# sine2pi/ASR-model

Measured on AMD Instinct MI355X. Metric: audio-sec/sec fwd+bwd on 30s@16kHz LibriSpeech-shaped clips (whole job, all GPUs), higher is better.
Workload: dtype bf16; 1 GPU; tiny (BASELINE configs[1]): log-mel + 4 enc/4 dec d=384 h=6 fwd+bwd, 32 x 30 s clips per GPU, T=256; model=tiny, global_batch=32, seq_len=3001, text_len=256, pitch_frames=3001, parallelism=dp1

## Files before the change

### asr-model_amd/csrc/gemm_wn.hip

```cpp
#include "gemm_wr.h"
#include "gemm_p2.h"
#include "gemm_ws.h"
#include <string>

static int g_wide_variant = 5;
static bool ws_on() { return (g_wide_variant & 4) != 0; }
static bool ws_any() { return (g_wide_variant & 8) != 0; }
extern "C" int asrx_set_gemm_variant(int v) {
  const int old = g_wide_variant;
  g_wide_variant = v;
  return old;
}
static bool p2_ok(const asrx::wn::Params& p, int conv, int nj, int a_bf16) {
  if (!a_bf16 && p.M >= 131072) return false;
  const bool vec = ((p.N | p.ldc) & 3) == 0 && ((uintptr_t)p.C & 15) == 0 && ((uintptr_t)p.Z & 15) == 0 &&
                   ((uintptr_t)p.Cb & 7) == 0;
  return (g_wide_variant & 3) >= 1 && !conv && (nj == 3 || nj == 2 || (nj == 1 && (g_wide_variant & 3) == 2)) &&
         vec && p.K >= 64;
}

namespace asrx {
namespace wn {

__global__ void weight_to_bf16_kernel(const float* __restrict__ src, unsigned short* __restrict__ dst, int rows,
                                      int cols, int64_t ld, int trans) {
  const int64_t total = (int64_t)rows * cols;
  for (int64_t i = (int64_t)blockIdx.x * blockDim.x + threadIdx.x; i < total; i += (int64_t)gridDim.x * blockDim.x) {
    int64_t r, c, o;
    if (!trans) {
      r = i / cols;
      c = i % cols;
      o = r * cols + c;
    } else {
      c = i / rows;
      r = i % rows;
      o = c * rows + r;
    }
    __bf16 h = (__bf16)src[r * ld + c];
    dst[o] = __builtin_bit_cast(unsigned short, h);
  }
}

}
}

using namespace asrx;

extern "C" int asrx_weight_to_bf16(const float* src, unsigned short* dst, int64_t rows, int64_t cols, int64_t ld,
                                   int trans, hipStream_t stream) {
  if (rows * cols == 0) return 0;
  const int64_t n = rows * cols;
  wn::weight_to_bf16_kernel<<<(unsigned)std::min<int64_t>((n + 255) / 256, 16384), 256, 0, stream>>>(
      src, dst, (int)rows, (int)cols, ld, trans);
  ASRX_LAUNCHED("asrx_weight_to_bf16");
}

struct WConv {
  const float* src;
  unsigned short* dst;
  int64_t ld;
  int rows, cols, trans, pad;
};

namespace asrx {
__global__ __launch_bounds__(256) void weights_to_bf16_kernel(const WConv* __restrict__ tab) {
  const WConv e = tab[blockIdx.y];
  const int64_t total = (int64_t)e.rows * e.cols;
  const int64_t i0 = (int64_t)blockIdx.x * 4096;
  if (i0 >= total) return;
  const int64_t i1 = min<int64_t>(total, i0 + 4096);
  for (int64_t i = i0 + threadIdx.x; i < i1; i += 256) {
    int64_t r, c, o;
    if (!e.trans) {
      r = i / e.cols;
      c = i % e.cols;
      o = r * e.cols + c;
    } else {
      c = i / e.rows;
      r = i % e.rows;
      o = c * e.rows + r;
    }
    e.dst[o] = __builtin_bit_cast(unsigned short, (__bf16)e.src[r * e.ld + c]);
  }
}
}

extern "C" int64_t asrx_wconv_entry_bytes(void) { return (int64_t)sizeof(WConv); }

extern "C" int asrx_weights_to_bf16(const void* tab, int64_t n, int64_t max_elems, hipStream_t stream) {
  if (n == 0) return 0;
  ASRX_REQUIRE(n < 65536, "asrx_weights_to_bf16: too many entries");
  dim3 grid((unsigned)((max_elems + 4095) / 4096), (unsigned)n);
  weights_to_bf16_kernel<<<grid, 256, 0, stream>>>((const WConv*)tab);
  ASRX_LAUNCHED("asrx_weights_to_bf16");
}

extern "C" int asrx_gemm_wn(const float* A, int64_t lda, int conv, int64_t convF, int64_t convC,
                            const unsigned short* W, int64_t ldw, float* C, int64_t ldc, const float* bias, float* Z,
                            int64_t M, int64_t N, int64_t K, float alpha, float beta, int act, int nj,
                            hipStream_t stream) {
  ASRX_REQUIRE(M > 0 && N > 0 && K > 0, "asrx_gemm_wn: empty problem");
  ASRX_REQUIRE(((uintptr_t)A & 15) == 0 && ((uintptr_t)W & 15) == 0, "asrx_gemm_wn: A/W must be 16-byte aligned");
  ASRX_REQUIRE(K % 8 == 0 && lda % 4 == 0 && ldw % 8 == 0, "asrx_gemm_wn: K%%8, lda%%4, ldw%%8 required");
  ASRX_REQUIRE(M * lda < (1LL << 31) && N * ldw < (1LL << 31), "asrx_gemm_wn: operand spans >= 2^31 elements");
  ASRX_REQUIRE(!conv || (convF > 0 && convC % 4 == 0), "asrx_gemm_wn: conv needs F > 0 and C %% 4 == 0");
  wn::Params p{A, (int)lda, W, (int)ldw, C, (int)ldc, bias, Z, (int)M, (int)N, (int)K,
               (int)(convF > 0 ? convF : 1), (int)(convC > 0 ? convC : 1), alpha, beta, act, nullptr, nullptr};
  if (nj == 3) conv ? wn::launch_wr<3, true>(p, stream) : wn::launch_wr<3, false>(p, stream);
  else if (nj == 2) conv ? wn::launch_wr<2, true>(p, stream) : wn::launch_wr<2, false>(p, stream);
  else conv ? wn::launch_wr<1, true>(p, stream) : wn::launch_wr<1, false>(p, stream);
  ASRX_LAUNCHED("asrx_gemm_wn");
}

extern "C" int asrx_gemm_wn_ex(const void* A, int a_bf16, int64_t lda, int conv, int64_t convF, int64_t convC,
                               const unsigned short* W, int64_t ldw, void* C, int c_bf16, int64_t ldc,
                               const float* bias, float* Z, int64_t M, int64_t N, int64_t K, float alpha, float beta,
                               int act, int nj, const int* mtiles, const int* n_mtiles, hipStream_t stream) {
  ASRX_REQUIRE(M > 0 && N > 0 && K > 0, "asrx_gemm_wn_ex: empty problem");
  ASRX_REQUIRE(((uintptr_t)A & 15) == 0 && ((uintptr_t)W & 15) == 0, "asrx_gemm_wn_ex: A/W must be 16-byte aligned");
  ASRX_REQUIRE(K % 8 == 0 && lda % (a_bf16 ? 8 : 4) == 0 && ldw % 8 == 0,
               "asrx_gemm_wn_ex: K%%8, lda%%4 (fp32) / lda%%8 (bf16), ldw%%8 required");
  ASRX_REQUIRE(M * lda < (1LL << 31) && N * ldw < (1LL << 31), "asrx_gemm_wn_ex: operand spans >= 2^31 elements");
  ASRX_REQUIRE(!conv || (convF > 0 && convC % (a_bf16 ? 8 : 4) == 0), "asrx_gemm_wn_ex: conv needs F > 0 and C %% 4 (8 for bf16)");
  ASRX_REQUIRE(!c_bf16 || beta == 0.f, "asrx_gemm_wn_ex: a bf16 output takes beta = 0");
  ASRX_REQUIRE(!(conv && mtiles), "asrx_gemm_wn_ex: tile lists are for plain GEMMs");
  wn::Params p{(const float*)A, (int)lda, W, (int)ldw, c_bf16 ? nullptr : (float*)C, (int)ldc, bias, Z, (int)M,
               (int)N, (int)K, (int)(convF > 0 ? convF : 1), (int)(convC > 0 ? convC : 1), alpha, beta, act,
               nullptr, nullptr, mtiles, n_mtiles, c_bf16 ? (unsigned short*)C : nullptr};
#define ASRX_WN_EX(NJV)                                                                              \
  if (a_bf16) conv ? wn::launch_wr<NJV, true, false, true>(p, stream) : wn::launch_wr<NJV, false, false, true>(p, stream); \
  else conv ? wn::launch_wr<NJV, true>(p, stream) : wn::launch_wr<NJV, false>(p, stream);
  if (ws_on() && !conv && wn::ws_ok(p, a_bf16, ws_any())) {
    a_bf16 ? wn::launch_ws_act<true>(p, stream) : wn::launch_ws_act<false>(p, stream);
  } else if (p2_ok(p, conv, nj, a_bf16)) {
    if (nj == 3) a_bf16 ? wn::launch_p2_act<3, true, false>(p, stream) : wn::launch_p2_act<3, false, false>(p, stream);
    else a_bf16 ? wn::launch_p2_act<2, true, false>(p, stream) : wn::launch_p2_act<2, false, false>(p, stream);
  } else if (nj == 3) { ASRX_WN_EX(3) }
  else if (nj == 2) { ASRX_WN_EX(2) }
  else { ASRX_WN_EX(1) }
#undef ASRX_WN_EX
  ASRX_LAUNCHED("asrx_gemm_wn_ex");
}

extern "C" int asrx_gemm_wn_ce(const void* A, int64_t lda, const unsigned short* W, int64_t ldw, unsigned short* Zb,
                               int64_t ldc, float* part, int64_t M, int64_t N, int64_t K, int nj, hipStream_t stream) {
  ASRX_REQUIRE(M > 0 && N > 0 && K > 0, "asrx_gemm_wn_ce: empty problem");
  ASRX_REQUIRE(((uintptr_t)A & 15) == 0 && ((uintptr_t)W & 15) == 0 && ((uintptr_t)Zb & 7) == 0 &&
                   ((uintptr_t)part & 7) == 0,
               "asrx_gemm_wn_ce: A/W 16-byte, Zb/part 8-byte aligned");
  ASRX_REQUIRE(K % 8 == 0 && lda % 8 == 0 && ldw % 8 == 0 && N % 4 == 0 && ldc % 4 == 0,
               "asrx_gemm_wn_ce: K, lda, ldw %% 8 and N, ldc %% 4 required");
  ASRX_REQUIRE(M * lda < (1LL << 31) && N * ldw < (1LL << 31), "asrx_gemm_wn_ce: operand spans >= 2^31 elements");
  ASRX_REQUIRE(nj >= 1 && nj <= 3, "asrx_gemm_wn_ce: nj in 1..3");
  wn::Params p{(const float*)A, (int)lda, W, (int)ldw, nullptr, (int)ldc, nullptr, nullptr, (int)M, (int)N, (int)K,
               1, 1, 1.f, 0.f, ACT_NONE, nullptr, nullptr, nullptr, nullptr, Zb, (float2*)part,
               (int)((N + 128 * nj - 1) / (128 * nj))};
  if (nj == 3) wn::launch_wr<3, false, false, true, true>(p, stream);
  else if (nj == 2) wn::launch_wr<2, false, false, true, true>(p, stream);
  else wn::launch_wr<1, false, false, true, true>(p, stream);
  ASRX_LAUNCHED("asrx_gemm_wn_ce");
}

extern "C" int asrx_gemm_wn_ce_f32(const void* A, int64_t lda, const unsigned short* W, int64_t ldw, float* Zf,
                               int64_t ldc, float* part, int64_t M, int64_t N, int64_t K, int nj, hipStream_t stream) {
  ASRX_REQUIRE(M > 0 && N > 0 && K > 0, "asrx_gemm_wn_ce_f32: empty problem");
  ASRX_REQUIRE(((uintptr_t)A & 15) == 0 && ((uintptr_t)W & 15) == 0 && ((uintptr_t)Zf & 15) == 0 &&
                   ((uintptr_t)part & 7) == 0,
               "asrx_gemm_wn_ce_f32: A/W 16-byte, Zf 16-byte, part 8-byte aligned");
  ASRX_REQUIRE(K % 8 == 0 && lda % 8 == 0 && ldw % 8 == 0 && N % 4 == 0 && ldc % 4 == 0,
               "asrx_gemm_wn_ce_f32: K, lda, ldw %% 8 and N, ldc %% 4 required");
  ASRX_REQUIRE(M * lda < (1LL << 31) && N * ldw < (1LL << 31), "asrx_gemm_wn_ce_f32: operand spans >= 2^31 elements");
  ASRX_REQUIRE(nj >= 1 && nj <= 3, "asrx_gemm_wn_ce_f32: nj in 1..3");
  wn::Params p{(const float*)A, (int)lda, W, (int)ldw, Zf, (int)ldc, nullptr, nullptr, (int)M, (int)N, (int)K,
               1, 1, 1.f, 0.f, ACT_NONE, nullptr, nullptr, nullptr, nullptr, nullptr, (float2*)part,
               (int)((N + 128 * nj - 1) / (128 * nj))};
  if (nj == 3) wn::launch_wr<3, false, false, true, true>(p, stream);
  else if (nj == 2) wn::launch_wr<2, false, false, true, true>(p, stream);
  else wn::launch_wr<1, false, false, true, true>(p, stream);
  ASRX_LAUNCHED("asrx_gemm_wn_ce_f32");
}

extern "C" int asrx_gemm_wn_head(const void* A, int64_t lda, const unsigned short* W, int64_t ldw, float* part,
                                 const int64_t* labels, float* zlab, int64_t M, int64_t N, int64_t K, int nj,
                                 hipStream_t stream) {
  ASRX_REQUIRE(M > 0 && N > 0 && K > 0, "asrx_gemm_wn_head: empty problem");
  ASRX_REQUIRE(((uintptr_t)A & 15) == 0 && ((uintptr_t)W & 15) == 0 && ((uintptr_t)part & 7) == 0,
               "asrx_gemm_wn_head: A/W 16-byte, part 8-byte aligned");
  ASRX_REQUIRE(K % 8 == 0 && lda % 8 == 0 && ldw % 8 == 0 && N % 4 == 0 && lda >= K,
               "asrx_gemm_wn_head: K, lda, ldw %% 8, N %% 4 and lda >= K required");
  ASRX_REQUIRE(M * lda < (1LL << 31) && N * ldw < (1LL << 31), "asrx_gemm_wn_head: operand spans >= 2^31 elements");
  ASRX_REQUIRE(nj >= 1 && nj <= 3, "asrx_gemm_wn_head: nj in 1..3");
  ASRX_REQUIRE(!labels || zlab, "asrx_gemm_wn_head: labels need zlab");
  const int64_t nparts = (N + 128 * nj - 1) / (128 * nj);
  wn::Params p{(const float*)A, (int)lda, W, (int)ldw, nullptr, (int)N, nullptr, nullptr, (int)M, (int)N, (int)K,
               1, 1, 1.f, 0.f, ACT_NONE, nullptr, nullptr, nullptr, nullptr, nullptr, (float2*)part, (int)nparts};
  p.hd_idx = reinterpret_cast<int*>(part + 2 * M * nparts);
  p.hd_labels = labels;
  p.hd_zlab = zlab;
  if (nj == 3) wn::launch_wr<3, false, false, true, true, false, false, false, true>(p, stream);
  else if (nj == 2) wn::launch_wr<2, false, false, true, true, false, false, false, true>(p, stream);
  else wn::launch_wr<1, false, false, true, true, false, false, false, true>(p, stream);
  ASRX_LAUNCHED("asrx_gemm_wn_head");
}

extern "C" int asrx_gemm_wn_res(const float* A, int64_t lda, const unsigned short* W, int64_t ldw, float* C, int64_t ldc,
                                const float* bias, const float* R, int64_t ldr, int64_t M, int64_t N, int64_t K, int nj,
                                hipStream_t stream) {
  ASRX_REQUIRE(M > 0 && N > 0 && K > 0, "asrx_gemm_wn_res: empty problem");
  ASRX_REQUIRE(((uintptr_t)A & 15) == 0 && ((uintptr_t)W & 15) == 0 && ((uintptr_t)C & 15) == 0 &&
                   ((uintptr_t)R & 15) == 0,
               "asrx_gemm_wn_res: A/W/C/R must be 16-byte aligned");
  ASRX_REQUIRE(K % 8 == 0 && lda % 4 == 0 && ldw % 8 == 0 && N % 4 == 0 && ldc % 4 == 0 && ldr % 4 == 0,
               "asrx_gemm_wn_res: K, ldw %% 8; lda, N, ldc, ldr %% 4");
  ASRX_REQUIRE(M * lda < (1LL << 31) && N * ldw < (1LL << 31), "asrx_gemm_wn_res: operand spans >= 2^31 elements");
  ASRX_REQUIRE(R && R != C, "asrx_gemm_wn_res: a residual input distinct from C is required");
  ASRX_REQUIRE(nj == 1 || nj == 3, "asrx_gemm_wn_res: nj 1 or 3");
  wn::Params p{A, (int)lda, W, (int)ldw, C, (int)ldc, bias, nullptr, (int)M, (int)N, (int)K, 1, 1, 1.f, 0.f,
               ACT_NONE, nullptr, nullptr, nullptr, nullptr, nullptr, nullptr, 0, R, (int)ldr};
  if (ws_on() && wn::ws_ok(p, false, ws_any())) wn::launch_ws<false, ACT_NONE, true, false>(p, stream);
  else if (nj == 3 && p2_ok(p, 0, nj, 0)) wn::launch_p2_act<3, false, true>(p, stream);
  else if (nj == 3) wn::launch_wr<3, false, false, false, false, true>(p, stream);
  else wn::launch_wr<1, false, false, false, false, true>(p, stream);
  ASRX_LAUNCHED("asrx_gemm_wn_res");
}

extern "C" int asrx_gemm_wn_rot(const void* A, int a_bf16, int64_t lda, const unsigned short* W, int64_t ldw,
                                float* C, float* Z, int64_t ldc, const float* bias, const float* m, const float* tab,
                                int64_t L, int64_t hd, float scale, int64_t M, int64_t N, int64_t K, int nj,
                                hipStream_t stream) {
  ASRX_REQUIRE(M > 0 && N > 0 && K > 0 && L > 0, "asrx_gemm_wn_rot: empty problem");
  ASRX_REQUIRE(((uintptr_t)A & 15) == 0 && ((uintptr_t)W & 15) == 0 && ((uintptr_t)C & 15) == 0 &&
                   ((uintptr_t)Z & 15) == 0 && ((uintptr_t)tab & 15) == 0,
               "asrx_gemm_wn_rot: A/W/C/Z/tab must be 16-byte aligned");
  ASRX_REQUIRE(K % 8 == 0 && lda % (a_bf16 ? 8 : 4) == 0 && ldw % 8 == 0 && N % 4 == 0 && ldc % 4 == 0,
               "asrx_gemm_wn_rot: K, ldw %% 8; lda %% 4 (8 bf16); N, ldc %% 4");
  ASRX_REQUIRE(hd >= 4 && hd % 4 == 0 && N % hd == 0, "asrx_gemm_wn_rot: head dim %% 4, N %% hd");
  ASRX_REQUIRE(M * lda < (1LL << 31) && N * ldw < (1LL << 31), "asrx_gemm_wn_rot: operand spans >= 2^31 elements");
  ASRX_REQUIRE(m && tab, "asrx_gemm_wn_rot: row norms and angle table required");
  ASRX_REQUIRE(nj == 1 || nj == 3, "asrx_gemm_wn_rot: nj 1 or 3");
  wn::Params p{(const float*)A, (int)lda, W, (int)ldw, C, (int)ldc, bias, Z, (int)M, (int)N, (int)K, 1, 1, 1.f, 0.f,
               ACT_NONE};
  p.rot_m = m;
  p.rot_tab = reinterpret_cast<const float2*>(tab);
  p.rot_L = (int)L;
  p.rot_half = (int)(hd / 2);
  p.rot_scale = scale;
  if (ws_on() && wn::ws_ok(p, a_bf16, ws_any())) a_bf16 ? wn::launch_ws<true, ACT_NONE, false, true>(p, stream)
                                      : wn::launch_ws<false, ACT_NONE, false, true>(p, stream);
  else if (nj == 3 && p2_ok(p, 0, nj, a_bf16)) a_bf16 ? wn::launch_p2<3, true, ACT_NONE, false, true>(p, stream)
                                                   : wn::launch_p2<3, false, ACT_NONE, false, true>(p, stream);
  else if (nj == 3) a_bf16 ? wn::launch_wr<3, false, false, true, false, false, false, true>(p, stream)
                           : wn::launch_wr<3, false, false, false, false, false, false, true>(p, stream);
  else a_bf16 ? wn::launch_wr<1, false, false, true, false, false, false, true>(p, stream)
              : wn::launch_wr<1, false, false, false, false, false, false, true>(p, stream);
  ASRX_LAUNCHED("asrx_gemm_wn_rot");
}

extern "C" int asrx_gemm_wn_gact(const void* A, int a_bf16, int64_t lda, const unsigned short* W, int64_t ldw,
                                 const float* bias, const float* G, int64_t ldg, unsigned short* gz, int64_t ldc,
                                 float* db, int64_t M, int64_t N, int64_t K, int act, int nj, hipStream_t stream) {
  ASRX_REQUIRE(M > 0 && N > 0 && K > 0, "asrx_gemm_wn_gact: empty problem");
  ASRX_REQUIRE(nj == 3, "asrx_gemm_wn_gact: nj 3 only");
  ASRX_REQUIRE(act == ACT_GELU || act == ACT_SILU || act == ACT_SIGMOID, "asrx_gemm_wn_gact: gelu/silu/sigmoid only");
  ASRX_REQUIRE(((uintptr_t)A & 15) == 0 && ((uintptr_t)W & 15) == 0 && ((uintptr_t)G & 15) == 0 &&
                   ((uintptr_t)gz & 7) == 0,
               "asrx_gemm_wn_gact: A/W/G 16-byte, gz 8-byte aligned");
  ASRX_REQUIRE(K % 8 == 0 && lda % (a_bf16 ? 8 : 4) == 0 && ldw % 8 == 0 && N % 4 == 0 && ldc % 4 == 0 &&
                   ldg % 4 == 0,
               "asrx_gemm_wn_gact: K, ldw %% 8; lda %% 4 (8 bf16); N, ldc, ldg %% 4");
  ASRX_REQUIRE(M * lda < (1LL << 31) && N * ldw < (1LL << 31), "asrx_gemm_wn_gact: operand spans >= 2^31 elements");
  wn::Params p{(const float*)A, (int)lda, W, (int)ldw, nullptr, (int)ldc, bias, nullptr, (int)M, (int)N, (int)K, 1,
               1, 1.f, 0.f, act, nullptr, nullptr, nullptr, nullptr, gz, nullptr, 0, nullptr, 0, G, (int)ldg, db};
  if (a_bf16) wn::launch_wr<3, false, false, true, false, false, true>(p, stream);
  else wn::launch_wr<3, false, false, false, false, false, true>(p, stream);
  ASRX_LAUNCHED("asrx_gemm_wn_gact");
}

extern "C" int asrx_gemm_wn_rows(const float* A, int64_t lda, const unsigned short* W, int64_t ldw, float* C,
                                 int64_t ldc, const float* bias, float* Z, int64_t M, int64_t N, int64_t K,
                                 float alpha, float beta, int act, int nj, const int* mtiles, const int* n_mtiles,
                                 hipStream_t stream) {
  ASRX_REQUIRE(M > 0 && N > 0 && K > 0, "asrx_gemm_wn_rows: empty problem");
  ASRX_REQUIRE(((uintptr_t)A & 15) == 0 && ((uintptr_t)W & 15) == 0, "asrx_gemm_wn_rows: A/W must be 16-byte aligned");
  ASRX_REQUIRE(K % 8 == 0 && lda % 4 == 0 && ldw % 8 == 0, "asrx_gemm_wn_rows: K%%8, lda%%4, ldw%%8 required");
  ASRX_REQUIRE(M * lda < (1LL << 31) && N * ldw < (1LL << 31), "asrx_gemm_wn_rows: operand spans >= 2^31 elements");
  ASRX_REQUIRE(mtiles && n_mtiles, "asrx_gemm_wn_rows: tile list required");
  wn::Params p{A, (int)lda, W, (int)ldw, C, (int)ldc, bias, Z, (int)M, (int)N, (int)K, 1, 1, alpha, beta, act,
               nullptr, nullptr, mtiles, n_mtiles};
  if (nj == 3) wn::launch_wr<3, false>(p, stream);
  else if (nj == 2) wn::launch_wr<2, false>(p, stream);
  else wn::launch_wr<1, false>(p, stream);
  ASRX_LAUNCHED("asrx_gemm_wn_rows");
}

namespace asrx {
__global__ __launch_bounds__(1024) void row_tiles_kernel(const float* __restrict__ next_i, int layer, int64_t L,
                                                         int64_t M, int* __restrict__ mtiles, int* __restrict__ n_out) {
  __shared__ int wsum[16];
  __shared__ int base;
  const int nm = (int)((M + wn::BM - 1) / wn::BM);
  if (threadIdx.x == 0) base = 0;
  __syncthreads();
  for (int t0 = 0; t0 < nm; t0 += 1024) {
    const int t = t0 + threadIdx.x;
    int act = 0;
    if (t < nm) {
      const int64_t r0 = (int64_t)t * wn::BM, r1 = min<int64_t>(r0 + wn::BM, M) - 1;
      for (int64_t b = r0 / L; b <= r1 / L && !act; ++b) act = next_i[b] == (float)layer;
    }
    const int lane = threadIdx.x & 63, w = threadIdx.x >> 6;
    int v = act;
    for (int o = 1; o < 64; o <<= 1) {
      const int u = __shfl_up(v, o);
      if (lane >= o) v += u;
    }
    if (lane == 63) wsum[w] = v;
    __syncthreads();
    int off = base;
    for (int k = 0; k < w; ++k) off += wsum[k];
    if (act) mtiles[off + v - 1] = t;
    __syncthreads();
    if (threadIdx.x == 0) {
      int tot = 0;
      for (int k = 0; k < 16; ++k) tot += wsum[k];
      base += tot;
    }
    __syncthreads();
  }
  if (threadIdx.x == 0) n_out[0] = base;
}
}

extern "C" int64_t asrx_row_tiles_max(int64_t M) { return (M + wn::BM - 1) / wn::BM; }

extern "C" int asrx_row_tiles(const float* next_i, int64_t layer, int64_t L, int64_t M, int* mtiles, int* n_mtiles,
                              hipStream_t stream) {
  ASRX_REQUIRE(L > 0 && M > 0, "asrx_row_tiles: empty");
  row_tiles_kernel<<<1, 1024, 0, stream>>>(next_i, (int)layer, L, M, mtiles, n_mtiles);
  ASRX_LAUNCHED("asrx_row_tiles");
}

namespace asrx {
namespace wn {

struct R64X {
  float4 v[4];
};
__global__ __launch_bounds__(256) void router64_kernel(Params p) {
  const int lane = threadIdx.x & 63, wid = threadIdx.x >> 6;
  const int lr = lane & 15, lk = lane >> 4;
  bf16x8 wf[4][2];
#pragma unroll
  for (int nb = 0; nb < 4; ++nb)
#pragma unroll
    for (int kb = 0; kb < 2; ++kb)
      wf[nb][kb] = *reinterpret_cast<const bf16x8*>(p.W + (int64_t)(16 * nb + lr) * p.ldw + 32 * kb + 8 * lk);
  float bv[4][4], w2v[3][4][4];
#pragma unroll
  for (int nb = 0; nb < 4; ++nb)
#pragma unroll
    for (int q = 0; q < 4; ++q) {
      const int n = 16 * nb + 4 * lk + q;
      bv[nb][q] = p.bias ? p.bias[n] : 0.f;
#pragma unroll
      for (int k = 0; k < 3; ++k) w2v[k][nb][q] = p.W2[k * 64 + n];
    }
  const int64_t ngroups = ((int64_t)p.M + 15) / 16;
  const int64_t step = (int64_t)gridDim.x * 4;
  const float* A = reinterpret_cast<const float*>(p.A);
  auto fetch = [&](int64_t g, R64X& x) __attribute__((always_inline)) {
    const int64_t row = min(g * 16 + lr, (int64_t)p.M - 1);
    const float* src = A + row * p.lda + 8 * lk;
    x.v[0] = *reinterpret_cast<const float4*>(src);
    x.v[1] = *reinterpret_cast<const float4*>(src + 4);
    x.v[2] = *reinterpret_cast<const float4*>(src + 32);
    x.v[3] = *reinterpret_cast<const float4*>(src + 36);
  };
  auto group = [&](int64_t g, const R64X& x) __attribute__((always_inline)) {
    bf16x8 xf[2];
#pragma unroll
    for (int kb = 0; kb < 2; ++kb) {
      const float4 a = x.v[2 * kb], b = x.v[2 * kb + 1];
      xf[kb] = bf16x8{(__bf16)a.x, (__bf16)a.y, (__bf16)a.z, (__bf16)a.w,
                      (__bf16)b.x, (__bf16)b.y, (__bf16)b.z, (__bf16)b.w};
    }
    f32x4 acc[4];
#pragma unroll
    for (int nb = 0; nb < 4; ++nb) acc[nb] = f32x4{0.f, 0.f, 0.f, 0.f};
#pragma unroll
    for (int kb = 0; kb < 2; ++kb)
#pragma unroll
      for (int nb = 0; nb < 4; ++nb) acc[nb] = __builtin_amdgcn_mfma_f32_16x16x32_bf16(wf[nb][kb], xf[kb], acc[nb], 0, 0, 0);
    const int64_t row = g * 16 + lr;
    float s[2][3];
#pragma unroll
    for (int grp = 0; grp < 2; ++grp) {
      float s0 = 0.f, s1 = 0.f, s2 = 0.f;
#pragma unroll
      for (int nt = 0; nt < 2; ++nt) {
        const int nb = 2 * grp + nt;
        const float v[4] = {p.alpha * acc[nb][0] + bv[nb][0], p.alpha * acc[nb][1] + bv[nb][1],
                            p.alpha * acc[nb][2] + bv[nb][2], p.alpha * acc[nb][3] + bv[nb][3]};
#pragma unroll
        for (int q = 0; q < 4; ++q) {
          const float h = silu_f(v[q]);
          s0 += h * w2v[0][nb][q];
          s1 += h * w2v[1][nb][q];
          s2 += h * w2v[2][nb][q];
        }
        if (p.C && row < p.M)
          *reinterpret_cast<float4*>(p.C + row * p.ldc + 16 * nb + 4 * lk) = make_float4(v[0], v[1], v[2], v[3]);
      }
      s0 += __shfl_xor(s0, 16); s1 += __shfl_xor(s1, 16); s2 += __shfl_xor(s2, 16);
      s0 += __shfl_xor(s0, 32); s1 += __shfl_xor(s1, 32); s2 += __shfl_xor(s2, 32);
      s[grp][0] = s0; s[grp][1] = s1; s[grp][2] = s2;
    }
    if (lk == 0 && row < p.M) {
#pragma unroll
      for (int k = 0; k < 3; ++k) p.R[row * 3 + k] = s[0][k] + s[1][k] + 0.f + 0.f;
    }
  };
  int64_t g = (int64_t)blockIdx.x * 4 + wid;
  if (g >= ngroups) return;
  R64X xa, xb;
  fetch(g, xa);
  fetch(g + step, xb);
  for (;; g += 2 * step) {
    {
      const R64X x = xa;
      fetch(g + 2 * step, xa);
      group(g, x);
    }
    if (g + step >= ngroups) break;
    {
      const R64X x = xb;
      fetch(g + 3 * step, xb);
      group(g + step, x);
    }
    if (g + 2 * step >= ngroups) break;
  }
}

}
}

extern "C" int asrx_gemm_wn_router(const float* A, int64_t lda, const unsigned short* W1, int64_t ldw,
                                   const float* b1, const float* W2, float* hpre, int64_t ldc, float* logits,
                                   int64_t M, int64_t N, int64_t K, hipStream_t stream) {
  ASRX_REQUIRE(M > 0 && N > 0 && K > 0, "asrx_gemm_wn_router: empty problem");
  ASRX_REQUIRE(N <= 384, "asrx_gemm_wn_router: N must be <= 384 (one tile column)");
  ASRX_REQUIRE(((uintptr_t)A & 15) == 0 && ((uintptr_t)W1 & 15) == 0, "asrx_gemm_wn_router: A/W must be 16-byte aligned");
  ASRX_REQUIRE(K % 8 == 0 && lda % 4 == 0 && ldw % 8 == 0, "asrx_gemm_wn_router: K%%8, lda%%4, ldw%%8 required");
  ASRX_REQUIRE(M * lda < (1LL << 31), "asrx_gemm_wn_router: operand spans >= 2^31 elements");
  wn::Params p{A, (int)lda, W1, (int)ldw, hpre, (int)ldc, b1, nullptr, (int)M, (int)N, (int)K, 1, 1, 1.f, 0.f,
               ACT_NONE, W2, logits};
  const bool r64 = N == 64 && K == 64 && W2 && (g_wide_variant & 16) == 0 && ldw % 8 == 0 &&
                   (!hpre || (ldc % 4 == 0 && ((uintptr_t)hpre & 15) == 0));
  if (r64) {
    static int cus = 0;
    if (!cus) {
      int dev = 0;
      (void)hipGetDevice(&dev);
      (void)hipDeviceGetAttribute(&cus, hipDeviceAttributeMultiprocessorCount, dev);
      cus = std::max(1, cus);
    }
    const int64_t groups = (M + 15) / 16;
    const unsigned grid = (unsigned)std::max<int64_t>(1, std::min<int64_t>((groups + 3) / 4, (int64_t)cus * 8));
    wn::router64_kernel<<<grid, 256, 0, stream>>>(p);
  } else if (N <= 128) wn::launch_wr<1, false, true>(p, stream);
  else if (N <= 256) wn::launch_wr<2, false, true>(p, stream);
  else wn::launch_wr<3, false, true>(p, stream);
  ASRX_LAUNCHED("asrx_gemm_wn_router");
}
```

Before: 5544 audio-sec/sec.

## Add persistent double-buffered bf16 GEMM kernel with direct global-to-LDS loads

Adds a persistent GEMM kernel for bf16 activations with nj==3. Each block walks several output tiles, double-buffers K-slabs in LDS using global_load_lds, and runs MFMA 16x16x32 on one buffer while the next slab loads. The bias-and-activation epilogue runs through LDS. It is on by default (variant 37) for large shapes (M>=8192, N>=384, K>=384), replacing the warp-specialized and p2 paths there. The aim is to hide load latency and cut launch and tail overhead, at the cost of a new code path with different tiling and occupancy.

```diff
diff --git a/asr-model_amd/csrc/gemm_pl.h b/asr-model_amd/csrc/gemm_pl.h
--- /dev/null
+++ b/asr-model_amd/csrc/gemm_pl.h
@@ -0,0 +1,211 @@
+#pragma once
+#include "gemm_wr.h"
+
+namespace asrx {
+namespace wn {
+
+namespace pl {
+constexpr int NTH = 256;
+constexpr int KS = 64;
+constexpr int BNP = 192;
+constexpr int A_IMG = BM * KS * 2;
+constexpr int W_IMG = BNP * KS * 2;
+constexpr int STAGE = A_IMG + W_IMG;
+constexpr int APC = A_IMG / 1024 / 4;
+constexpr int WPC = W_IMG / 1024 / 4;
+constexpr int SLAB = 4 * EpLds<3>::FLOATS * 4;
+static_assert(SLAB + BNP * 4 <= STAGE, "slab and bias slice fit in one stage buffer");
+typedef __attribute__((address_space(3))) char lds_char;
+typedef const __attribute__((address_space(1))) char gl_char;
+}
+
+#ifndef PL_ABL
+#define PL_ABL 0
+#endif
+
+#define ASRX_PL_BARRIER()                            \
+  do {                                               \
+    asm volatile("s_waitcnt lgkmcnt(0)" ::: "memory"); \
+    __builtin_amdgcn_s_barrier();                    \
+    asm volatile("" ::: "memory");                   \
+  } while (0)
+
+template <int ACT>
+__global__ __launch_bounds__(pl::NTH, 2) void gemm_pl_kernel(Params p, int ntiles) {
+  using namespace pl;
+  __shared__ __attribute__((aligned(1024))) char lds[2 * STAGE];
+
+  const int nN = (p.N + BNP - 1) / BNP;
+  const int nk = p.K / KS;
+  const int G = gridDim.x, bid = blockIdx.x;
+  const int r = (G % 8 == 0) ? (bid & 7) * (G >> 3) + (bid >> 3) : bid;
+  const int my = r < ntiles ? (ntiles - r + G - 1) / G : 0;
+  const int S = my * nk;
+  const int tid = threadIdx.x, lane = tid & 63;
+  const int wid = __builtin_amdgcn_readfirstlane(tid >> 6);
+  const int wm = wid >> 1, wn = wid & 1;
+  const int lr = lane & 15, lk = lane >> 4;
+
+  int lj = 0, lkk = 0;
+  uint32_t oa[APC], ow[WPC];
+  auto enter = [&]() __attribute__((always_inline)) {
+    const int t = lj * G + r;
+    const int tm = t / nN;
+    const int m0 = tm * BM, n0 = (t - tm * nN) * BNP;
+#pragma unroll
+    for (int i = 0; i < APC; ++i) {
+      const int row = 8 * (wid + 4 * i) + (lane >> 3);
+      const int c = (lane & 7) ^ sw64(row);
+      oa[i] = (uint32_t)(((int64_t)min(m0 + row, p.M - 1) * p.lda + 8 * c) * 2);
+    }
+#pragma unroll
+    for (int i = 0; i < WPC; ++i) {
+      const int row = 8 * (wid + 4 * (APC + i)) + (lane >> 3) - BM;
+      const int c = (lane & 7) ^ sw64(row);
+      ow[i] = (uint32_t)(((int64_t)min(n0 + row, p.N - 1) * p.ldw + 8 * c) * 2);
+    }
+  };
+  auto issue = [&](int buf) __attribute__((always_inline)) {
+#if !(PL_ABL & 1)
+    gl_char* Ab = (gl_char*)(reinterpret_cast<const char*>(p.A) + (size_t)lkk * (KS * 2));
+    gl_char* Wb = (gl_char*)(reinterpret_cast<const char*>(p.W) + (size_t)lkk * (KS * 2));
+    lds_char* dst = (lds_char*)lds + buf * STAGE + wid * 1024;
+#pragma unroll
+    for (int i = 0; i < APC; ++i) __builtin_amdgcn_global_load_lds(Ab + oa[i], dst + 4096 * i, 16, 0, 0);
+#pragma unroll
+    for (int i = 0; i < WPC; ++i) __builtin_amdgcn_global_load_lds(Wb + ow[i], dst + 4096 * (APC + i), 16, 0, 0);
+#endif
+    if (++lkk == nk) {
+      lkk = 0;
+      ++lj;
+      enter();
+    }
+  };
+
+  int fa[4], fb[6];
+#pragma unroll
+  for (int mt = 0; mt < 4; ++mt) {
+    const int rr = wm * 64 + mt * 16 + lr;
+    fa[mt] = rr * 128 + 16 * (lk ^ sw64(rr));
+  }
+#pragma unroll
+  for (int nt = 0; nt < 6; ++nt) {
+    const int n = wn * 96 + nt * 16 + lr;
+    fb[nt] = A_IMG + n * 128 + 16 * (lk ^ sw64(n));
+  }
+
+  f32x4 acc[4][6];
+#pragma unroll
+  for (int i = 0; i < 4; ++i)
+#pragma unroll
+    for (int j = 0; j < 6; ++j) acc[i][j] = f32x4{0.f, 0.f, 0.f, 0.f};
+
+  if (S == 0) return;
+  enter();
+  issue(0);
+  asm volatile("s_waitcnt vmcnt(0)" ::: "memory");
+  ASRX_PL_BARRIER();
+
+  int ej = 0, ekk = 0;
+  for (int s = 0; s < S; ++s) {
+    const int buf = s & 1;
+    if (s + 1 < S) issue(buf ^ 1);
+    const bool last = ekk == nk - 1;
+    int m0 = 0, n0 = 0;
+    float bv = 0.f;
+    if (last) {
+      const int t = ej * G + r;
+      const int tm = t / nN;
+      m0 = tm * BM;
+      n0 = (t - tm * nN) * BNP;
+      const float* bp = p.bias ? p.bias + min(n0 + min(tid, BNP - 1), p.N - 1) : reinterpret_cast<const float*>(p.W);
+      asm volatile("global_load_dword %0, %1, off" : "=v"(bv) : "v"(bp) : "memory");
+    }
+    const char* St = lds + buf * STAGE;
+#pragma unroll
+    for (int h = 0; h < 2; ++h) {
+      bf16x8 a[4], b[6];
+#pragma unroll
+      for (int mt = 0; mt < 4; ++mt) a[mt] = *reinterpret_cast<const bf16x8*>(St + (fa[mt] ^ (64 * h)));
+#pragma unroll
+      for (int nt = 0; nt < 6; ++nt) b[nt] = *reinterpret_cast<const bf16x8*>(St + (fb[nt] ^ (64 * h)));
+      __builtin_amdgcn_s_setprio(1);
+#pragma unroll
+      for (int mt = 0; mt < 4; ++mt)
+#pragma unroll
+        for (int nt = 0; nt < 6; ++nt)
+#if !(PL_ABL & 4)
+          acc[mt][nt] = __builtin_amdgcn_mfma_f32_16x16x32_bf16(b[nt], a[mt], acc[mt][nt], 0, 0, 0);
+#else
+          acc[mt][nt][0] += (float)a[mt][0] * (float)b[nt][0];
+#endif
+      __builtin_amdgcn_s_setprio(0);
+    }
+    asm volatile("s_waitcnt vmcnt(0)" ::: "memory");
+    ASRX_PL_BARRIER();
+    if (last) {
+      float* bias_s = reinterpret_cast<float*>(lds + buf * STAGE + SLAB);
+      if (tid < BNP) bias_s[tid] = bv;
+      ASRX_PL_BARRIER();
+#if !(PL_ABL & 8)
+      float* ep = reinterpret_cast<float*>(lds + buf * STAGE) + wid * EpLds<3>::FLOATS;
+      epilogue_lds<3, ACT, false, false>(p, acc, bias_s, m0, n0, wm, wn, lr, lk, ep);
+#else
+      {
+        float t = 0.f;
+#pragma unroll
+        for (int i = 0; i < 4; ++i)
+#pragma unroll
+          for (int q = 0; q < 6; ++q) t += acc[i][q][0] + acc[i][q][1] + acc[i][q][2] + acc[i][q][3];
+        if (t == 1.2345e-37f) p.C[m0] = t;
+      }
+#endif
+#pragma unroll
+      for (int i = 0; i < 4; ++i)
+#pragma unroll
+        for (int q = 0; q < 6; ++q) acc[i][q] = f32x4{0.f, 0.f, 0.f, 0.f};
+      ekk = 0;
+      ++ej;
+      ASRX_PL_BARRIER();
+    } else {
+      ++ekk;
+    }
+  }
+}
+
+inline bool pl_can(const Params& p, int a_bf16, int conv, int nj) {
+  const bool vec = ((p.N | p.ldc) & 3) == 0 && ((uintptr_t)p.C & 15) == 0 && ((uintptr_t)p.Z & 15) == 0 &&
+                   ((uintptr_t)p.Cb & 7) == 0;
+  return a_bf16 && !conv && nj == 3 && !p.mtiles && p.K % pl::KS == 0 && vec &&
+         (uint64_t)p.M * p.lda * 2 < (1ull << 32) && (uint64_t)p.N * p.ldw * 2 < (1ull << 32);
+}
+
+template <int ACT>
+void launch_pl(const Params& p, hipStream_t s) {
+  static int resident = 0;
+  if (!resident) {
+    int per_cu = 0, dev = 0, cus = 0;
+    (void)hipOccupancyMaxActiveBlocksPerMultiprocessor(&per_cu, (const void*)gemm_pl_kernel<ACT>, pl::NTH, 0);
+    (void)hipGetDevice(&dev);
+    (void)hipDeviceGetAttribute(&cus, hipDeviceAttributeMultiprocessorCount, dev);
+    resident = std::max(1, per_cu) * std::max(1, cus);
+  }
+  const int tiles = ((p.M + BM - 1) / BM) * ((p.N + pl::BNP - 1) / pl::BNP);
+  gemm_pl_kernel<ACT><<<std::min(tiles, resident), pl::NTH, 0, s>>>(p, tiles);
+}
+
+}
+}
+
+#ifndef ASRX_PL_INSTANTIATE
+#define ASRX_PL_DECL(ACT) extern template void asrx::wn::launch_pl<ACT>(const asrx::wn::Params&, hipStream_t);
+#else
+#define ASRX_PL_DECL(ACT) template void asrx::wn::launch_pl<ACT>(const asrx::wn::Params&, hipStream_t);
+#endif
+#ifndef ASRX_PL_INSTANTIATE
+ASRX_PL_DECL(asrx::ACT_NONE)
+ASRX_PL_DECL(asrx::ACT_GELU)
+ASRX_PL_DECL(asrx::ACT_SILU)
+ASRX_PL_DECL(asrx::ACT_SIGMOID)
+ASRX_PL_DECL(asrx::ACT_RELU)
+#endif
diff --git a/asr-model_amd/csrc/gemm_pl_a.hip b/asr-model_amd/csrc/gemm_pl_a.hip
--- /dev/null
+++ b/asr-model_amd/csrc/gemm_pl_a.hip
@@ -0,0 +1,5 @@
+#define ASRX_PL_INSTANTIATE
+#include "gemm_pl.h"
+
+ASRX_PL_DECL(asrx::ACT_NONE)
+ASRX_PL_DECL(asrx::ACT_RELU)
diff --git a/asr-model_amd/csrc/gemm_pl_b.hip b/asr-model_amd/csrc/gemm_pl_b.hip
--- /dev/null
+++ b/asr-model_amd/csrc/gemm_pl_b.hip
@@ -0,0 +1,6 @@
+#define ASRX_PL_INSTANTIATE
+#include "gemm_pl.h"
+
+ASRX_PL_DECL(asrx::ACT_GELU)
+ASRX_PL_DECL(asrx::ACT_SILU)
+ASRX_PL_DECL(asrx::ACT_SIGMOID)
diff --git a/asr-model_amd/csrc/gemm_wn.hip b/asr-model_amd/csrc/gemm_wn.hip
--- a/asr-model_amd/csrc/gemm_wn.hip
+++ b/asr-model_amd/csrc/gemm_wn.hip
@@ -1,9 +1,10 @@
 #include "gemm_wr.h"
 #include "gemm_p2.h"
 #include "gemm_ws.h"
+#include "gemm_pl.h"
 #include <string>
 
-static int g_wide_variant = 5;
+static int g_wide_variant = 37;
 static bool ws_on() { return (g_wide_variant & 4) != 0; }
 static bool ws_any() { return (g_wide_variant & 8) != 0; }
 extern "C" int asrx_set_gemm_variant(int v) {
@@ -17,6 +18,23 @@
                    ((uintptr_t)p.Cb & 7) == 0;
   return (g_wide_variant & 3) >= 1 && !conv && (nj == 3 || nj == 2 || (nj == 1 && (g_wide_variant & 3) == 2)) &&
          vec && p.K >= 64;
+}
+
+static void launch_pl_act(const asrx::wn::Params& p, hipStream_t s) {
+  using namespace asrx;
+  switch (p.act) {
+    case ACT_GELU: wn::launch_pl<ACT_GELU>(p, s); break;
+    case ACT_SILU: wn::launch_pl<ACT_SILU>(p, s); break;
+    case ACT_SIGMOID: wn::launch_pl<ACT_SIGMOID>(p, s); break;
+    case ACT_RELU: wn::launch_pl<ACT_RELU>(p, s); break;
+    default: wn::launch_pl<ACT_NONE>(p, s); break;
+  }
+}
+
+static bool pl_measured(const asrx::wn::Params& p) { return p.M >= 8192 && p.N >= 384 && p.K >= 384; }
+static bool pl_ok(const asrx::wn::Params& p, int a_bf16, int conv, int nj) {
+  if ((g_wide_variant & (32 | 64)) == 0 || !asrx::wn::pl_can(p, a_bf16, conv, nj)) return false;
+  return (g_wide_variant & 64) != 0 || pl_measured(p);
 }
 
 namespace asrx {
@@ -130,7 +148,9 @@
 #define ASRX_WN_EX(NJV)                                                                              \
   if (a_bf16) conv ? wn::launch_wr<NJV, true, false, true>(p, stream) : wn::launch_wr<NJV, false, false, true>(p, stream); \
   else conv ? wn::launch_wr<NJV, true>(p, stream) : wn::launch_wr<NJV, false>(p, stream);
-  if (ws_on() && !conv && wn::ws_ok(p, a_bf16, ws_any())) {
+  if (pl_ok(p, a_bf16, conv, nj)) {
+    launch_pl_act(p, stream);
+  } else if (ws_on() && !conv && wn::ws_ok(p, a_bf16, ws_any())) {
     a_bf16 ? wn::launch_ws_act<true>(p, stream) : wn::launch_ws_act<false>(p, stream);
   } else if (p2_ok(p, conv, nj, a_bf16)) {
     if (nj == 3) a_bf16 ? wn::launch_p2_act<3, true, false>(p, stream) : wn::launch_p2_act<3, false, false>(p, stream);
```

Result: no change. 5589 audio-sec/sec (median of 6 runs) (+0.8%).
